# Denys88/rl_games

Hardware: AMD Instinct MI355X
Metric: ppo_env_steps_per_sec (higher is better)
Workload: dtype f32

## Files before the change

rl_games_amd/csrc/mlp_chain_bx_fwd.hip:

```cpp

#ifndef RLG_BX_FWD_W
#define RLG_BX_FWD_W 8
#endif
#if RLG_BX_FWD_W == 8 && !defined(RLG_ACC_CLASS)
#define RLG_ACC_CLASS "+v"
#endif
#ifndef RLG_BX_FWD_NF
#define RLG_BX_FWD_NF (RLG_BX_FWD_W == 8 ? 1 : 2)
#endif

#include "mlp_chain_bx.hpp"
#include "mlp_chain_shared.hpp"

namespace rlg {

constexpr int kFwG = 4;
constexpr int kFwUnitBlocks = RLG_BX_FWD_NF;
constexpr int kFwW = RLG_BX_FWD_W;
static_assert(kFwW % kFwG == 0, "the prologue deals row group (wave % G) to a wave");
constexpr int kFwMaxPersist = 16 / kFwW;

template <int G, int NF>
__device__ __forceinline__ void bx_span(rsrc_t pr, unsigned layer_off, int KC, const char* tile_lane, int ob_first, int nb_valid,
                                        int c0, int c1, f32x4 (&acc)[NF][G], bool first) {
  const unsigned lane16 = static_cast<unsigned>(lane_id()) * 16u;
  int boff[NF];
#pragma unroll
  for (int f = 0; f < NF; ++f) {
    const int ob = ob_first + (f < nb_valid ? f : nb_valid - 1);
    boff[f] = __builtin_amdgcn_readfirstlane(static_cast<int>(layer_off) + ob * KC * kBxChunk);
  }
  u32x4 a0[NF][kBxPlanes], a1[NF][kBxPlanes], b0[G][kBxPlanes], b1[G][kBxPlanes];
  auto load_a = [&](u32x4 (&av)[NF][kBxPlanes], int c) {
#pragma unroll
    for (int f = 0; f < NF; ++f) {
#pragma unroll
      for (int p = 0; p < kBxPlanes; ++p)
        av[f][p] = __builtin_bit_cast(u32x4, __builtin_amdgcn_raw_buffer_load_b128(pr, lane16 + static_cast<unsigned>(p * kBxFrag),
                                                                                  boff[f] + c * kBxChunk, 0));
    }
  };
  auto load_b = [&](u32x4 (&bv)[G][kBxPlanes], int c) {
    const char* p = tile_lane + c * G * kBxChunk;
#pragma unroll
    for (int g = 0; g < G; ++g) {
#pragma unroll
      for (int pl = 0; pl < kBxPlanes; ++pl) bv[g][pl] = *reinterpret_cast<const u32x4*>(p + (g * kBxPlanes + pl) * kBxFrag);
    }
  };
  auto mfmas = [&](auto first_tag, const u32x4 (&av)[NF][kBxPlanes], const u32x4 (&bv)[G][kBxPlanes]) {
    constexpr bool kFirst = decltype(first_tag)::value;
#pragma unroll
    for (int f = 0; f < NF; ++f) {
#pragma unroll
      for (int g = 0; g < G; ++g) {
#pragma unroll
        for (int t = 0; t < kBxProducts; ++t)
          acc[f][g] = bx_mfma(av[f][kBxPa[t]], bv[g][kBxPb[t]], (kFirst && t == 0) ? f32x4{0.0f, 0.0f, 0.0f, 0.0f} : acc[f][g]);
        asm volatile("" : RLG_ACC_REG(acc[f][g]));
      }
    }
  };
  auto step = [&](auto cur_tag, auto pf_tag, int c, auto first_tag) {
    constexpr bool kCur1 = decltype(cur_tag)::value;
    constexpr bool kPf = decltype(pf_tag)::value;
    if constexpr (kPf) {
      load_a(kCur1 ? a0 : a1, c + 1);
      load_b(kCur1 ? b0 : b1, c + 1);
    }
    mfmas(first_tag, kCur1 ? a1 : a0, kCur1 ? b1 : b0);
    if constexpr (kPf) {
#pragma unroll
      for (int i = 0; i < kBxPlanes * NF; ++i) {
        __builtin_amdgcn_sched_group_barrier(0x008, 1, 0);
        __builtin_amdgcn_sched_group_barrier(0x020, 1, 0);
      }
#pragma unroll
      for (int i = 0; i < kBxPlanes * G; ++i) {
        __builtin_amdgcn_sched_group_barrier(0x008, 1, 0);
        __builtin_amdgcn_sched_group_barrier(0x100, 1, 0);
      }
      if constexpr (kBxProducts * NF * G - kBxPlanes * (NF + G) > 0)
        __builtin_amdgcn_sched_group_barrier(0x008, kBxProducts * NF * G - kBxPlanes * (NF + G), 0);
    }
    RLG_PIN();
  };
  constexpr std::true_type T{};
  constexpr std::false_type F{};
  load_a(a0, c0);
  load_b(b0, c0);
  int c = c0;
  if (c + 1 < c1) {
    if (first) step(F, T, c, T);
    else step(F, T, c, F);
  } else {
    if (first) step(F, F, c, T);
    else step(F, F, c, F);
    return;
  }
  ++c;
  for (; c + 2 < c1; c += 2) {
    step(T, T, c, F);
    step(F, T, c + 1, F);
  }
  if (c1 - c == 2) {
    step(T, T, c, F);
    step(F, F, c + 1, F);
  } else {
    step(T, F, c, F);
  }
}

template <int HACT>
__global__ __launch_bounds__(64 * kFwW) void mlp_chain_fwd_bx_kernel(ChainArgs a) {
  constexpr int G = kFwG, W = kFwW;
  extern __shared__ __attribute__((aligned(16))) float lds[];
  if (static_cast<int>(blockIdx.x) >= a.fwd_blocks) {
    if (threadIdx.x < 256) chain_pack_planes_block(a.pack, static_cast<int>(blockIdx.x) - a.fwd_blocks, threadIdx.x);
    return;
  }
  char* const ldsb = reinterpret_cast<char*>(lds);
  const int lane = lane_id();
  const int wave = wave_id_uniform();
  const int q4 = 4 * (lane >> 4);
  const long long row0 = static_cast<long long>(blockIdx.x) * (16 * G);
  const rsrc_t pr = make_rsrc(a.planes, a.planes_bytes);
  const int num_layers = pin_s(a.num_layers);
  const long long n_rows = pin_s(a.rows);
  int stamp = 0;
  chain_stamp(a.dbg, wave, stamp);

  float scale_in[G];
#pragma unroll
  for (int g = 0; g < G; ++g) scale_in[g] = kBxScaleObsNorm;
  {
    const int in0 = a.layer[0].in;
    const int in0p = (in0 + 3) & ~3;
    const bool norm = a.rms_mean != nullptr;
    const int KC0 = (in0 + 31) >> 5;
    const int nfrag = KC0 * G;
    const bool xv = vec4_ok(a.x, a.ldx);
    const bool xnv = a.xn != nullptr && vec4_ok(a.xn, in0);
    float* stats = reinterpret_cast<float*>(ldsb + a.bx_stats_off);
    char* t0 = ldsb + a.bx_tile_off[0];
    constexpr int kProBatch = 4;
    f32x4 xlo[kProBatch], xhi[kProBatch];
    const bool fast = pin_s(static_cast<int>(xv && (in0 & 3) == 0 && a.ldx * 64 * 4 < static_cast<long long>(kOob))) != 0;
    const rsrc_t xr = make_rsrc(a.x + row0 * a.ldx, fast ? tile_bytes(n_rows - row0, 16 * G, a.ldx) : 0u);
    const unsigned x_lane = static_cast<unsigned>(((lane & 15) * static_cast<int>(a.ldx) + q4) * 4);
    const unsigned x_group = static_cast<unsigned>(16 * static_cast<int>(a.ldx) * 4);
    auto load_frags = [&](int u0) {
#pragma unroll
      for (int k = 0; k < kProBatch; ++k) {
        const int u = u0 + k * W;
        const int c = u / G, g = u - c * G;
        const long long row = row0 + g * 16 + (lane & 15);
        xlo[k] = xhi[k] = f32x4{0.0f, 0.0f, 0.0f, 0.0f};
        if (fast) {
          const unsigned off = x_lane + static_cast<unsigned>(g) * x_group + static_cast<unsigned>(c) * 128u;
          xlo[k] = buf_load4(xr, (u < nfrag && c * 32 + q4 < in0) ? off : kOob);
          xhi[k] = buf_load4(xr, (u < nfrag && c * 32 + 16 + q4 < in0) ? off + 64u : kOob);
        } else if (u < nfrag && row < n_rows) {
          xlo[k] = load_row4(a.x, a.ldx, row, c * 32 + q4, in0, xv);
          xhi[k] = load_row4(a.x, a.ldx, row, c * 32 + 16 + q4, in0, xv);
        }
      }
    };
    auto put_frags = [&](int u0, float scale) {
#pragma unroll
      for (int k = 0; k < kProBatch; ++k) {
        const int u = u0 + k * W;
        if (u < nfrag) {
          const int c = u / G, g = u - c * G;
          const long long row = row0 + g * 16 + (lane & 15);
          f32x4 v[2] = {xlo[k], xhi[k]};
#pragma unroll
          for (int h = 0; h < 2; ++h) {
            const int f = c * 32 + 16 * h + q4;
            if (fast) {
              if (norm && f < in0) {
                const f32x4 m4 = *reinterpret_cast<const f32x4*>(stats + f);
                const f32x4 d4 = *reinterpret_cast<const f32x4*>(stats + in0p + f);
#pragma unroll
                for (int e = 0; e < 4; ++e) v[h][e] = clamp_nan((v[h][e] - m4[e]) / d4[e], -5.0f, 5.0f);
                if (row >= n_rows) v[h] = f32x4{0.0f, 0.0f, 0.0f, 0.0f};
              }
              if (a.xn && f < in0 && row < n_rows) store_row4(a.xn, in0, row, f, in0, v[h], xnv);
            } else if (row < n_rows) {
              if (norm) {
#pragma unroll
                for (int e = 0; e < 4; ++e) {
                  if (f + e < in0) v[h][e] = clamp_nan((v[h][e] - stats[f + e]) / stats[in0p + f + e], -5.0f, 5.0f);
                }
              }
              if (a.xn && f < in0) store_row4(a.xn, in0, row, f, in0, v[h], xnv);
            }
          }
          const float x[8] = {v[0][0], v[0][1], v[0][2], v[0][3], v[1][0], v[1][1], v[1][2], v[1][3]};
          u32x4 plane[kBxPlanes];
          bx_split8(x, scale, plane);
#pragma unroll
          for (int p = 0; p < kBxPlanes; ++p) *reinterpret_cast<u32x4*>(t0 + (u * kBxPlanes + p) * kBxFrag + lane * 16) = plane[p];
        }
      }
    };
    load_frags(wave);
    chain_stamp(a.dbg, wave, stamp);
    if (norm) {
      chain_norm_stats<W>(a, stats, in0, in0p);
      chain_stamp(a.dbg, wave, stamp);
      __syncthreads();
    }
    chain_stamp(a.dbg, wave, stamp);
    float scale_mine = kBxScaleObsNorm;
    if (RLG_BX_F16 && !norm) {
      float mine = 0.0f;
      const int group = wave % G;
      const long long row = row0 + group * 16 + (lane & 15);
      if (row < n_rows) {
        for (int c = 0; c < KC0; ++c) {
          const f32x4 lo = load_row4(a.x, a.ldx, row, c * 32 + q4, in0, xv), hi = load_row4(a.x, a.ldx, row, c * 32 + 16 + q4, in0, xv);
#pragma unroll
          for (int e = 0; e < 4; ++e) mine = __builtin_fmaxf(mine, __builtin_fmaxf(bx_finite_abs(lo[e]), bx_finite_abs(hi[e])));
        }
      }
      scale_mine = bx_row_scale(mine);
      if (lane < 16 && wave < G) stats[group * 16 + lane] = scale_mine;
    }
    put_frags(wave, scale_mine);
    for (int u0 = wave + W * kProBatch; u0 < nfrag; u0 += W * kProBatch) {
      load_frags(u0);
      put_frags(u0, scale_mine);
    }
    __syncthreads();
    if (RLG_BX_F16 && !norm) {
#pragma unroll
      for (int g = 0; g < G; ++g) scale_in[g] = stats[g * 16 + (lane & 15)];
      __syncthreads();
    }
  }
  chain_stamp(a.dbg, wave, stamp);

  auto wave_blocks = [&](int nob) -> int { return nob / W + (wave < nob % W ? 1 : 0); };
  auto wave_first = [&](int nob) -> int { return wave * (nob / W) + (wave < nob % W ? wave : nob % W); };
  const int pass_layer = pin_s(a.bx_pass_layer), win = pin_s(a.bx_pass_chunks);
  f32x4 bval[kFwUnitBlocks], bnext[kFwUnitBlocks];

  for (int L = 0; L < num_layers; ++L) {
    const bool last = (L == num_layers - 1);
    const int l_in = pin_s(a.layer[L].in), l_out = pin_s(a.layer[L].out);
    const int KC = (l_in + 31) >> 5, NOB = (l_out + 15) >> 4;
    const unsigned l_off = static_cast<unsigned>(pin_s(static_cast<int>(a.p_off[L])));
    const char* tin = ldsb + pin_s(a.bx_tile_off[L]);
    char* tout = last ? nullptr : ldsb + pin_s(a.bx_tile_off[L + 1]);

    auto make_epilogue = [&](int layer, char* dst_tile, int chunk_base, const float (&in_scale)[G]) {
      const int width = pin_s(a.layer[layer].out), act = pin_s(a.layer[layer].act);
      float* ph = pin_s(a.layer[layer].h);
      const long long ld = pin_s(a.layer[layer].ldh);
      const bool h_on = ph != nullptr;
      const rsrc_t hr = make_rsrc(h_on ? ph + row0 * ld : nullptr, h_on ? tile_bytes(n_rows - row0, 16 * G, ld) : 0u);
      const unsigned h_lane = static_cast<unsigned>(((lane & 15) * static_cast<int>(ld) + q4) * 4);
      const unsigned h_group = static_cast<unsigned>(16 * static_cast<int>(ld) * 4);
      const bool h_fast = pin_s(static_cast<int>(h_on && vec4_ok(ph, ld) && (width & 3) == 0)) != 0;
      float inv[G];
#pragma unroll
      for (int g = 0; g < G; ++g) inv[g] = 1.0f / (kBxScaleW * in_scale[g]);
      return [=](int ob, int g, const f32x4& accv, const f32x4& bias) {
        const int f = ob * 16 + q4;
        f32x4 z;
        if constexpr (RLG_BX_F16) {
#pragma unroll
          for (int e = 0; e < 4; ++e) z[e] = __builtin_fmaf(accv[e], inv[g], bias[e]);
        } else {
          z = accv + bias;
        }
        const f32x4 v = chain_act4<HACT>(z, act);
        if (h_on) {
          const unsigned off = h_lane + static_cast<unsigned>(g) * h_group + static_cast<unsigned>(ob) * 64u;
          if (h_fast) {
            buf_store4(hr, f < width ? off : kOob, v);
          } else {
#pragma unroll
            for (int e = 0; e < 4; ++e) buf_store1(hr, f + e < width ? off + 4u * e : kOob, v[e]);
          }
        }
        if (dst_tile != nullptr) {
          unsigned plane[kBxPlanes][2];
          bx_split4(v, kBxScaleH, plane);
          char* dst = dst_tile + ((((ob >> 1) - chunk_base) * G + g) * kBxPlanes) * kBxFrag + lane * 16 + (ob & 1) * 8;
#pragma unroll
          for (int p = 0; p < kBxPlanes; ++p) *reinterpret_cast<uint2*>(dst + p * kBxFrag) = make_uint2(plane[p][0], plane[p][1]);
        }
      };
    };
    auto bias_rsrc = [&](int layer) -> rsrc_t {
      return make_rsrc(pin_s(a.layer[layer].bias), static_cast<unsigned>(pin_s(a.layer[layer].out)) * 4u);
    };
    auto load_bias = [&](rsrc_t br, int fo, bool fast) -> f32x4 {
      if (fast) return buf_load4(br, static_cast<unsigned>(fo) * 4u);
      f32x4 v;
#pragma unroll
      for (int e = 0; e < 4; ++e) v[e] = buf_load1(br, static_cast<unsigned>(fo + e) * 4u);
      return v;
    };
    auto bias_fast = [&](int layer) -> bool {
      return pin_s(static_cast<int>(aligned16(a.layer[layer].bias) && (a.layer[layer].out & 3) == 0)) != 0;
    };
    auto run_blocks = [&](int b0, int b1, char* dst_tile, int chunk_base) {
      const int nb = b1 - b0;
      const int nb_w = wave_blocks(nb), first_ob = b0 + wave_first(nb);
      const int unitsw = (kFwUnitBlocks > 2) ? nb_w / kFwUnitBlocks : 0;
      const int rest = nb_w - kFwUnitBlocks * unitsw;
      const int units2 = (kFwUnitBlocks == 3 || kFwUnitBlocks == 1) ? 0 : rest >> 1, left = rest - 2 * units2;
      const rsrc_t br = bias_rsrc(L);
      const bool bfast = bias_fast(L);
      auto epilogue = make_epilogue(L, dst_tile, chunk_base, scale_in);
      auto whole = [&](auto nf_tag, int first, int nunits) {
        constexpr int NF = decltype(nf_tag)::value;
        bx_units<G, G, NF>(
            pr, l_off, KC, tin + lane * 16, nunits, [&](int j) { return first + j * NF; }, [&](int) { return 0; },
            [&](int j) {
#pragma unroll
              for (int f = 0; f < NF; ++f) {
                const int fo = (first + (j < nunits ? j : nunits - 1) * NF + f) * 16 + q4;
                bnext[f] = load_bias(br, fo, bfast);
              }
            },
            [&]() {
#pragma unroll
              for (int f = 0; f < NF; ++f) {
                bval[f] = bnext[f];
                asm volatile("" : "+v"(bval[f]));
              }
            },
            [&](int j, const f32x4 (&acc)[NF][G]) {
#pragma unroll
              for (int f = 0; f < NF; ++f) {
#pragma unroll
                for (int g = 0; g < G; ++g) epilogue(first + j * NF + f, g, acc[f][g], bval[f]);
              }
            },
            false);
      };
      if constexpr (kFwUnitBlocks > 2) whole(std::integral_constant<int, kFwUnitBlocks>{}, first_ob, unitsw);
      if constexpr (kFwUnitBlocks != 3 && kFwUnitBlocks != 1)
        whole(std::integral_constant<int, 2>{}, first_ob + kFwUnitBlocks * unitsw, units2);
      whole(std::integral_constant<int, 1>{}, first_ob + kFwUnitBlocks * unitsw + 2 * units2, left);
    };
    auto zero_pad = [&](char* tile, int nob, int chunk_base) {
      if (tile != nullptr && (nob & 1)) {
        for (int u = wave; u < G * kBxPlanes; u += W)
          *reinterpret_cast<uint2*>(tile + ((((nob >> 1) - chunk_base) * G) * kBxPlanes + u) * kBxFrag + lane * 16 + 8) = make_uint2(0u, 0u);
      }
    };

    if (L + 1 != pass_layer) {
      run_blocks(0, NOB, tout, 0);
      zero_pad(tout, NOB, 0);
      chain_stamp(a.dbg, wave, stamp);
      __syncthreads();
      chain_stamp(a.dbg, wave, stamp);
#pragma unroll
      for (int g = 0; g < G; ++g) scale_in[g] = kBxScaleH;
      continue;
    }

    const int P = L + 1;
    const int p_in = pin_s(a.layer[P].in), p_out = pin_s(a.layer[P].out);
    const int KCP = (p_in + 31) >> 5, NOBP = (p_out + 15) >> 4;
    const unsigned p_off = static_cast<unsigned>(pin_s(static_cast<int>(a.p_off[P])));
    const int pnb = wave_blocks(NOBP), pfirst = wave_first(NOBP);
    const bool p_last = (P == num_layers - 1);
    char* ptile = p_last ? nullptr : ldsb + pin_s(a.bx_tile_off[P + 1]);
    f32x4 pacc[kFwMaxPersist][G];
    for (int c0 = 0; c0 < KCP; c0 += win) {
      const int c1 = (c0 + win < KCP) ? c0 + win : KCP;
      const int b0 = 2 * c0, b1 = (2 * c1 < NOB) ? 2 * c1 : NOB;
      run_blocks(b0, b1, tout, c0);
      if (b1 == NOB) zero_pad(tout, NOB, c0);
      __syncthreads();
      if (pnb > 0) bx_span<G, kFwMaxPersist>(pr, p_off, KCP, tout + lane * 16 - c0 * G * kBxChunk, pfirst, pnb, c0, c1, pacc, c0 == 0);
      __syncthreads();
    }
    chain_stamp(a.dbg, wave, stamp);
    if (pnb > 0) {
      const rsrc_t br = bias_rsrc(P);
      const bool bfast = bias_fast(P);
      float hidden_scale[G];
#pragma unroll
      for (int g = 0; g < G; ++g) hidden_scale[g] = kBxScaleH;
      auto epilogue = make_epilogue(P, ptile, 0, hidden_scale);
      f32x4 pb[kFwMaxPersist];
#pragma unroll
      for (int f = 0; f < kFwMaxPersist; ++f) {
        const int fo = (pfirst + f) * 16 + q4;
        pb[f] = load_bias(br, f < pnb ? fo : p_out, bfast);
      }
      asm volatile("s_nop 7" : RLG_ACC_REG(pacc[0][0]));
#pragma unroll
      for (int f = 0; f < kFwMaxPersist; ++f) {
        if (f < pnb) {
#pragma unroll
          for (int g = 0; g < G; ++g) epilogue(pfirst + f, g, pacc[f][g], pb[f]);
        }
      }
    }
    zero_pad(ptile, NOBP, 0);
    chain_stamp(a.dbg, wave, stamp);
    __syncthreads();
    chain_stamp(a.dbg, wave, stamp);
#pragma unroll
    for (int g = 0; g < G; ++g) scale_in[g] = kBxScaleH;
    ++L;
  }
}

int chain_bx_fwd_plan(ChainArgs& args) {
  const int n = args.num_layers;
  long long kc[kChainMaxLayers];
  for (int L = 0; L < n; ++L) kc[L] = bx_kc(args.layer[L].in);
  const long long chunk = kFwG * kBxChunk;
  long long stats = ((2LL * ((args.layer[0].in + 3) & ~3) * 4) + 15) & ~15LL;
  if (stats < 16 * kFwG * 4) stats = 16 * kFwG * 4;
  long long need = kc[0] * chunk + stats;
  for (int L = 0; L < n; ++L) {
    const long long pair = (kc[L] + (L + 1 < n ? kc[L + 1] : 0)) * chunk;
    need = pair > need ? pair : need;
  }
  const long long budget = need <= 160 * 1024 ? need : 160 * 1024;
  auto place = [&](int p, long long window) -> bool {
    for (int L = 0; L < n; ++L) {
      const long long c = (L == p) ? window : kc[L];
      if (c * chunk > budget) return false;
      args.bx_tile_off[L] = static_cast<int>((L & 1) ? budget - c * chunk : 0);
    }
    args.bx_tile_off[n] = 0;
    for (int L = 0; L + 1 < n; ++L) {
      if (L == p) continue;
      const long long c0 = kc[L], c1 = (L + 1 == p) ? window : kc[L + 1];
      if ((c0 + c1) * chunk > budget) return false;
    }
    if (kc[0] * chunk + stats > budget) return false;
    args.bx_stats_off = static_cast<int>(budget - stats);
    return true;
  };
  args.bx_pass_layer = -1;
  args.bx_pass_chunks = 0;
  if (place(-1, 0)) return static_cast<int>(budget);
  int p = -1;
  for (int L = 1; L < n; ++L) {
    if (p < 0 || kc[L] > kc[p]) p = L;
  }
  if (p < 1) return -1;
  if (bx_nb(args.layer[p].out) > kFwMaxPersist * kFwW) return -1;
  for (long long passes = 2; passes <= kc[p]; ++passes) {
    const long long window = (kc[p] + passes - 1) / passes;
    if (place(p, window)) {
      args.bx_pass_layer = p;
      args.bx_pass_chunks = static_cast<int>(window);
      return static_cast<int>(budget);
    }
  }
  return -1;
}

bool chain_bx_fwd_eligible(const ChainArgs& args) {
  if (args.planes == nullptr) return false;
  for (int L = 0; L < args.num_layers; ++L) {
    const ChainLayer& ly = args.layer[L];
    if (reinterpret_cast<uintptr_t>(ly.bias) & 3u) return false;
    if (ly.h != nullptr && ly.ldh * 64 * 4 >= static_cast<long long>(kOob)) return false;
  }
  return true;
}

template <int HACT>
static int chain_bx_launch_fwd_as(const ChainArgs& args_in, int lds_bytes, hipStream_t st, hipEvent_t ev0, hipEvent_t ev1) {
  ChainArgs args = args_in;
  int grid = static_cast<int>((args.rows + 16 * kFwG - 1) / (16 * kFwG));
  args.fwd_blocks = grid;
  if (args.pack.total_pairs > 0) grid += chain_bx_pack_blocks(args.pack);
  return chain_launch_timed(mlp_chain_fwd_bx_kernel<HACT>, grid, 64 * kFwW, lds_bytes, st, ev0, ev1, args);
}
int chain_bx_fwd_prepare() {
  static bool raised = false;
  if (raised) return 0;
  for (const void* k : {reinterpret_cast<const void*>(mlp_chain_fwd_bx_kernel<kChElu>),
                        reinterpret_cast<const void*>(mlp_chain_fwd_bx_kernel<kChAny>)}) {
    const hipError_t e = hipFuncSetAttribute(k, hipFuncAttributeMaxDynamicSharedMemorySize, 160 * 1024);
    if (e != hipSuccess) return static_cast<int>(e);
  }
  raised = true;
  return 0;
}
int chain_bx_launch_fwd(const ChainArgs& args, int lds_bytes, hipStream_t st, hipEvent_t ev0, hipEvent_t ev1) {
  if (const int e = chain_bx_fwd_prepare()) return e;
  return chain_elu_only(args) ? chain_bx_launch_fwd_as<kChElu>(args, lds_bytes, st, ev0, ev1)
                  : chain_bx_launch_fwd_as<kChAny>(args, lds_bytes, st, ev0, ev1);
}

}
```

Before: 26.47 million.

## Prefetch weights for short ELU layers before the barrier and run one block per wave

Adds a fast path for small layers that follow a normal layer (at most 4 K-chunks, and output blocks times row groups fit within the wave count). Each wave issues its weight and bias buffer loads for the next layer before the __syncthreads, then computes a single 16-row by 16-column block from LDS and applies the epilogue. The aim is to hide global-load latency behind the barrier and to skip the general span and scheduling machinery for small layers. The cost is more registers for the prefetched fragments, and waves outside the layer's block count do redundant loads while idle.

```diff
diff --git a/rl_games_amd/csrc/mlp_chain_bx_fwd.hip b/rl_games_amd/csrc/mlp_chain_bx_fwd.hip
--- a/rl_games_amd/csrc/mlp_chain_bx_fwd.hip
+++ b/rl_games_amd/csrc/mlp_chain_bx_fwd.hip
@@ -19,6 +19,10 @@
 constexpr int kFwW = RLG_BX_FWD_W;
 static_assert(kFwW % kFwG == 0, "the prologue deals row group (wave % G) to a wave");
 constexpr int kFwMaxPersist = 16 / kFwW;
+#ifndef RLG_BX_PRIME
+#define RLG_BX_PRIME 1
+#endif
+constexpr int kFwShortKC = 4;
 
 template <int G, int NF>
 __device__ __forceinline__ void bx_span(rsrc_t pr, unsigned layer_off, int KC, const char* tile_lane, int ob_first, int nb_valid,
@@ -109,6 +113,23 @@
   } else {
     step(T, F, c, F);
   }
+}
+
+template <int KCMAX>
+__device__ __forceinline__ f32x4 bx_short_span(const u32x4 (&pre_a)[KCMAX][kBxPlanes], int KC, const char* tile_lane_group) {
+  f32x4 acc = {0.0f, 0.0f, 0.0f, 0.0f};
+#pragma unroll
+  for (int c = 0; c < KCMAX; ++c) {
+    if (c < KC) {
+      u32x4 b[kBxPlanes];
+#pragma unroll
+      for (int p = 0; p < kBxPlanes; ++p) b[p] = *reinterpret_cast<const u32x4*>(tile_lane_group + c * kFwG * kBxChunk + p * kBxFrag);
+#pragma unroll
+      for (int t = 0; t < kBxProducts; ++t) acc = bx_mfma(pre_a[c][kBxPa[t]], b[kBxPb[t]], acc);
+    }
+  }
+  asm volatile("s_nop 7" : RLG_ACC_REG(acc));
+  return acc;
 }
 
 template <int HACT>
@@ -245,6 +266,10 @@
   auto wave_first = [&](int nob) -> int { return wave * (nob / W) + (wave < nob % W ? wave : nob % W); };
   const int pass_layer = pin_s(a.bx_pass_layer), win = pin_s(a.bx_pass_chunks);
   f32x4 bval[kFwUnitBlocks], bnext[kFwUnitBlocks];
+  auto short_shape = [&](int l, int kc, int nob) -> bool {
+    if (RLG_BX_PRIME == 0 || HACT != kChElu || l < 1 || l >= num_layers || (pass_layer >= 0 && l >= pass_layer - 1 && l <= pass_layer + 1)) return false;
+    return kc <= kFwShortKC && nob * G <= W;
+  };
 
   for (int L = 0; L < num_layers; ++L) {
     const bool last = (L == num_layers - 1);
@@ -266,7 +291,7 @@
       float inv[G];
 #pragma unroll
       for (int g = 0; g < G; ++g) inv[g] = 1.0f / (kBxScaleW * in_scale[g]);
-      return [=](int ob, int g, const f32x4& accv, const f32x4& bias) {
+      return [=](int ob, int g, const f32x4& accv, const f32x4& bias) __attribute__((always_inline)) {
         const int f = ob * 16 + q4;
         f32x4 z;
         if constexpr (RLG_BX_F16) {
@@ -358,6 +383,40 @@
     if (L + 1 != pass_layer) {
       run_blocks(0, NOB, tout, 0);
       zero_pad(tout, NOB, 0);
+      while (L + 1 < num_layers) {
+        const int S = L + 1;
+        const int kcs = (pin_s(a.layer[S].in) + 31) >> 5, nobs = (pin_s(a.layer[S].out) + 15) >> 4;
+        if (!short_shape(S, kcs, nobs)) break;
+        const int s_off = pin_s(static_cast<int>(a.p_off[S]));
+        const rsrc_t s_br = bias_rsrc(S);
+        const bool s_bfast = bias_fast(S);
+        const bool mine = wave < nobs * G;
+        const int ob = mine ? wave / G : nobs - 1, g = wave % G;
+        u32x4 pre_a[kFwShortKC][kBxPlanes];
+        const int off = s_off + ob * kcs * kBxChunk;
+#pragma unroll
+        for (int c = 0; c < kFwShortKC; ++c) {
+#pragma unroll
+          for (int p = 0; p < kBxPlanes; ++p)
+            pre_a[c][p] = __builtin_bit_cast(u32x4, __builtin_amdgcn_raw_buffer_load_b128(pr, static_cast<unsigned>(lane * 16 + p * kBxFrag),
+                                                                                         off + (c < kcs ? c : kcs - 1) * kBxChunk, 0));
+        }
+        const f32x4 pre_bias = load_bias(s_br, ob * 16 + q4, s_bfast);
+        chain_stamp(a.dbg, wave, stamp);
+        __syncthreads();
+        chain_stamp(a.dbg, wave, stamp);
+#pragma unroll
+        for (int gg = 0; gg < G; ++gg) scale_in[gg] = kBxScaleH;
+        char* touts = (S == num_layers - 1) ? nullptr : ldsb + pin_s(a.bx_tile_off[S + 1]);
+        auto epilogue = make_epilogue(S, touts, 0, scale_in);
+        const f32x4 acc = bx_short_span<kFwShortKC>(pre_a, kcs, ldsb + pin_s(a.bx_tile_off[S]) + lane * 16 + g * kBxChunk);
+#pragma unroll
+        for (int gg = 0; gg < G; ++gg) {
+          if (mine && gg == g) epilogue(ob, gg, acc, pre_bias);
+        }
+        ++L;
+        zero_pad(touts, nobs, 0);
+      }
       chain_stamp(a.dbg, wave, stamp);
       __syncthreads();
       chain_stamp(a.dbg, wave, stamp);
```

After: 26.20 million. 0.99x the previous value.
